# vsois/hanabi-agents

Hardware: AMD Instinct MI355X
Metric: env_steps_per_sec (higher is better)
Workload: dtype u8 env/encoder + bfloat16 Q-net GEMM (fp32 accumulate, fp32 master weights)

## Files before the change

hanabi-agents_amd/csrc/actor_fused.hip:

```cpp
#include <hip/hip_runtime.h>
#include <hip/hip_bf16.h>
#include <hip/hip_fp16.h>

#include <cstdint>
#include <type_traits>

#include "../../include/hanabi_hip.h"
#include "common.hpp"
#include "env_kernel.hpp"

using hb::fail;

namespace {

typedef __bf16 bf16x8 __attribute__((ext_vector_type(8)));
typedef _Float16 f16x8 __attribute__((ext_vector_type(8)));
typedef float f32x4 __attribute__((ext_vector_type(4)));

constexpr int FM = 128;
constexpr int FH = 512;
constexpr int FNT = 512;
constexpr int FK = 51;
constexpr int S2 = FH / 32;
constexpr int LUT_BYTES = 65536;
constexpr int H_BYTES = FM * FH * 2;
constexpr int FRAG_FLOATS = 3 * 8 * FM;
constexpr int LDS_TOTAL = H_BYTES + FRAG_FLOATS * 4;
constexpr float NEG_BIG = -1e30f;

struct FusedArgs {
  const uint32_t* obs;
  long long m;
  int words;
  int s1;
  const uint4* w1f;
  const float* b1;
  const uint4* w2f;
  const float* b2;
  const float* support;
  float* q;
  int n_actions, n_pass;
  const int8_t* legal;
  int32_t* actions;
  float epsilon;
  unsigned long long seed, draw;
  long long first_gid;
  unsigned long long* stamps;
};

#ifdef HB_STAMPS
#define HB_FSTAMP(slot)                                                                              \
  do {                                                                                               \
    __builtin_amdgcn_sched_barrier(0);                                                               \
    unsigned long long hb_t_;                                                                        \
    asm volatile("s_memtime %0\n\ts_waitcnt lgkmcnt(0)" : "=s"(hb_t_)::"memory");                    \
    if (a.stamps && lane == 0) a.stamps[(static_cast<long long>(blockIdx.x) * 8 + wave) * 16 + (slot)] = hb_t_; \
    __builtin_amdgcn_sched_barrier(0);                                                               \
  } while (0)
#define HB_FSTAMP_REAL(slot)                                                                         \
  do {                                                                                               \
    unsigned long long hb_t_;                                                                        \
    asm volatile("s_memrealtime %0\n\ts_waitcnt lgkmcnt(0)" : "=s"(hb_t_)::"memory");                \
    if (a.stamps && lane == 0) a.stamps[(static_cast<long long>(blockIdx.x) * 8 + wave) * 16 + (slot)] = hb_t_; \
  } while (0)
#else
#define HB_FSTAMP(slot) do {} while (0)
#define HB_FSTAMP_REAL(slot) do {} while (0)
#endif

template <bool F16>
__device__ __forceinline__ uint32_t pack16(float lo, float hi) {
  if constexpr (F16) {
    const _Float16 a = static_cast<_Float16>(lo), b = static_cast<_Float16>(hi);
    uint16_t ua, ub;
    __builtin_memcpy(&ua, &a, 2);
    __builtin_memcpy(&ub, &b, 2);
    return static_cast<uint32_t>(ua) | (static_cast<uint32_t>(ub) << 16);
  } else {
    const __hip_bfloat16 a = __float2bfloat16(lo), b = __float2bfloat16(hi);
    return static_cast<uint32_t>(*reinterpret_cast<const uint16_t*>(&a)) |
           (static_cast<uint32_t>(*reinterpret_cast<const uint16_t*>(&b)) << 16);
  }
}
template <bool F16>
__device__ __forceinline__ uint32_t bits2_one(uint32_t b, int p) {
  const uint32_t t = (b >> (2 * p)) & 3u;
  return __umul24((t | (t << 15)) & 0x00010001u, F16 ? 0x3C00u : 0x3F80u);
}
template <bool F16>
__device__ __forceinline__ f32x4 mfma16(const uint4& wv, const uint4& xv, const f32x4& c) {
  if constexpr (F16) {
    union { uint4 u; f16x8 f; } w, x;
    w.u = wv; x.u = xv;
    return __builtin_amdgcn_mfma_f32_16x16x32_f16(w.f, x.f, c, 0, 0, 0);
  } else {
    union { uint4 u; bf16x8 f; } w, x;
    w.u = wv; x.u = xv;
    return __builtin_amdgcn_mfma_f32_16x16x32_bf16(w.f, x.f, c, 0, 0, 0);
  }
}
typedef float f32x2 __attribute__((ext_vector_type(2)));
typedef unsigned int u32x2 __attribute__((ext_vector_type(2)));
__device__ __forceinline__ float vmax(float a, float b) {
  float r;
  asm("v_max_f32 %0, %1, %2" : "=v"(r) : "v"(a), "v"(b));
  return r;
}
__device__ __forceinline__ float vmax3(float a, float b, float c) {
  float r;
  asm("v_max3_f32 %0, %1, %2, %3" : "=v"(r) : "v"(a), "v"(b), "v"(c));
  return r;
}
__device__ __forceinline__ float exp2_fast(float x) { return __builtin_amdgcn_exp2f(x); }

template <bool F16, class K, int EG>
__device__ __forceinline__ void actor_fused_body(const FusedArgs& a) {
  __shared__ __attribute__((aligned(16))) unsigned char lds[LDS_TOTAL];
  const int tid = threadIdx.x, lane = tid & 63;
  const int wave = __builtin_amdgcn_readfirstlane(tid >> 6);
  const int r = lane & 15, qd = lane >> 4;
  const long long row0 = static_cast<long long>(blockIdx.x) * FM;
  const int s1 = a.s1, G = (s1 + 3) >> 2;
  unsigned char* lutb = lds + (LDS_TOTAL - LUT_BYTES);
  const int bits_off = LDS_TOTAL - LUT_BYTES - 2048 * G;
  unsigned char* bits = lds + bits_off;
  const int m_early = bits_off >> 14;

  HB_FSTAMP_REAL(14);
  HB_FSTAMP(0);
  const uint4* w1p = a.w1f + (4 * wave) * 64 + lane;
  uint4 wa[4], wb[4];
#pragma unroll
  for (int n = 0; n < 4; ++n) wa[n] = w1p[n * 64];

  uint32_t w[4] = {0u, 0u, 0u, 0u};
  auto load_item = [&](int it) {
    const int rr = it & (FM - 1), g = it >> 7;
    long long row = row0 + rr;
    if (row >= a.m) row = a.m - 1;
    const uint32_t* src = a.obs + row * a.words + 4 * g;
#pragma unroll
    for (int i = 0; i < 4; ++i) w[i] = (4 * g + i < a.words) ? src[i] : 0u;
  };
  if (tid < FM * G) load_item(tid);
  for (int e = tid; e < 4096; e += FNT) {
    const uint32_t v = static_cast<uint32_t>(e) >> 4;
    *reinterpret_cast<uint4*>(lutb + e * 16) = make_uint4(bits2_one<F16>(v, 0), bits2_one<F16>(v, 1), bits2_one<F16>(v, 2), bits2_one<F16>(v, 3));
  }
  for (int it = tid; it < FM * G; it += FNT) {
    const int rr = it & (FM - 1), g = it >> 7;
    if (it != tid) load_item(it);
    uint32_t* dst = reinterpret_cast<uint32_t*>(bits) + (static_cast<size_t>((rr >> 4) * G + g) * 64 + (rr & 15));
#pragma unroll
    for (int qq = 0; qq < 4; ++qq) {
      const uint32_t o = ((w[0] >> (8 * qq)) & 0xFFu) | (((w[1] >> (8 * qq)) & 0xFFu) << 8) | (((w[2] >> (8 * qq)) & 0xFFu) << 16) |
                         (((w[3] >> (8 * qq)) & 0xFFu) << 24);
      dst[qq * 16] = o;
    }
  }
  HB_FSTAMP(1);
  __syncthreads();
  HB_FSTAMP(2);

  f32x4 acc[4][8];
#pragma unroll
  for (int n = 0; n < 4; ++n) {
    const float4 b = *reinterpret_cast<const float4*>(a.b1 + 64 * wave + 16 * n + 4 * qd);
#pragma unroll
    for (int m = 0; m < 8; ++m) acc[n][m] = f32x4{b.x, b.y, b.z, b.w};
  }

  {
    const unsigned char* lut = lutb + r * 16;
    const uint32_t* bw = reinterpret_cast<const uint32_t*>(bits) + lane;
#define HB_L1_STEP(I, WCUR, WNXT, HAVE_NEXT)                                                                   \
  {                                                                                                            \
    const int s_ = 4 * g + (I);                                                                                \
    if (HAVE_NEXT) {                                                                                           \
      _Pragma("unroll") for (int n = 0; n < 4; ++n) WNXT[n] = w1p[(s_ + 1) * 2048 + n * 64];                    \
    }                                                                                                          \
    asm volatile("" ::: "memory");                \
    uint4 xf[8];                                                                                               \
    _Pragma("unroll") for (int m = 0; m < 8; ++m) {                                                            \
      const uint32_t v = (xw[m] >> (8 * (I))) & 0xFFu;                                                         \
      xf[m] = *reinterpret_cast<const uint4*>(lut + v * 256u);                                                 \
    }                                                                                                          \
    _Pragma("unroll") for (int n = 0; n < 4; ++n) {                                                            \
      _Pragma("unroll") for (int m = 0; m < 8; ++m)                                                            \
        acc[n][m] = mfma16<F16>(WCUR[n], xf[m], acc[n][m]);                                                    \
    }                                                                                                          \
  }
    for (int g = 0; g < G; ++g) {
      uint32_t xw[8];
#pragma unroll
      for (int m = 0; m < 8; ++m) xw[m] = bw[(m * G + g) * 64];
      HB_L1_STEP(0, wa, wb, true)
      const bool more = 4 * g + 2 < s1;
      HB_L1_STEP(1, wb, wa, more)
      if (more) {
        HB_L1_STEP(2, wa, wb, true)
        HB_L1_STEP(3, wb, wa, (4 * g + 4 < s1))
      }
// ... 74 lines not shown
#undef HB_L2_HALF
    if (p < 2) HB_FSTAMP(7 + 3 * p);
    if (p + 1 < n_pass) {
#pragma unroll
      for (int n = 0; n < 4; ++n) wa[n] = wp[S2 * 2048 + n * 64];
    }

    auto sup_at = [&](int k) { return a.support[k < FK ? k : FK - 1]; };
    f32x2 supF[6];
#pragma unroll
    for (int i = 0; i < 6; ++i) supF[i] = f32x2{sup_at(4 * (2 * i) + qd), sup_at(4 * (2 * i + 1) + qd)};
    const float supF12 = sup_at(48 + qd);
    const int fq = wave & 3;
    const f32x2 supZa = f32x2{sup_at(13 * fq + qd), sup_at(13 * fq + 4 + qd)};
    const f32x2 supZb = f32x2{sup_at(13 * fq + 8 + qd), sup_at(13 * fq + 12)};
    const bool full_ok = slot < A && slot < full_cap;
    float* fb = reinterpret_cast<float*>(lds + H_BYTES) + wave * FM;
    const f32x2 L2 = f32x2{LOG2E, LOG2E};
    hb::static_for<2>([&](auto MH) {
    constexpr int M0 = 4 * decltype(MH)::value;
    float qF[4], zm[4], zs[4], zt[4], vf12[4], vz3[4], nmx[4], nmz[4];
#define HB_M for (int m = 0; m < 4; ++m)
#define HB_SWAP16(X, OP) { const u32x2 t_ = __builtin_amdgcn_permlane16_swap(__float_as_uint(X), __float_as_uint(X), false, false); \
                           X = OP(__uint_as_float(t_.x), __uint_as_float(t_.y)); }
#define HB_SWAP32(X, OP) { const u32x2 t_ = __builtin_amdgcn_permlane32_swap(__float_as_uint(X), __float_as_uint(X), false, false); \
                           X = OP(__uint_as_float(t_.x), __uint_as_float(t_.y)); }
#define HB_ADD(A_, B_) ((A_) + (B_))
#pragma unroll
    HB_M { vf12[m] = qd < 3 ? acc[3][M0 + m][0] : NEG_BIG; vz3[m] = qd == 3 ? acc[3][M0 + m][0] : NEG_BIG; }
#pragma unroll
    HB_M nmx[m] = vmax3(acc[0][M0 + m][0], acc[0][M0 + m][1], acc[0][M0 + m][2]);
#pragma unroll
    HB_M nmx[m] = vmax3(nmx[m], acc[0][M0 + m][3], acc[1][M0 + m][0]);
#pragma unroll
    HB_M nmx[m] = vmax3(nmx[m], acc[1][M0 + m][1], acc[1][M0 + m][2]);
#pragma unroll
    HB_M nmx[m] = vmax3(nmx[m], acc[1][M0 + m][3], acc[2][M0 + m][0]);
#pragma unroll
    HB_M nmx[m] = vmax3(nmx[m], acc[2][M0 + m][1], acc[2][M0 + m][2]);
#pragma unroll
    HB_M nmx[m] = vmax3(nmx[m], acc[2][M0 + m][3], vf12[m]);
#pragma unroll
    HB_M nmz[m] = vmax(vmax3(acc[3][M0 + m][1], acc[3][M0 + m][2], acc[3][M0 + m][3]), vz3[m]);
#pragma unroll
    HB_M HB_SWAP16(nmx[m], vmax)
#pragma unroll
    HB_M HB_SWAP16(nmz[m], vmax)
#pragma unroll
    HB_M HB_SWAP32(nmx[m], vmax)
#pragma unroll
    HB_M HB_SWAP32(nmz[m], vmax)
#pragma unroll
    HB_M { nmx[m] *= -LOG2E; nmz[m] *= -LOG2E; }
    f32x2 s2[4], t2[4];
#define HB_PAIR_FIRST(N, LO, SUP)                                                                   \
  _Pragma("unroll") HB_M {                                                                          \
    const f32x2 arg = f32x2{acc[N][M0 + m][LO], acc[N][M0 + m][LO + 1]} * L2 + f32x2{nmx[m], nmx[m]};         \
    const f32x2 e = f32x2{exp2_fast(arg.x), exp2_fast(arg.y)};                                      \
    s2[m] = e;                                                                                      \
    t2[m] = e * SUP;                                                                                \
  }
#define HB_PAIR(N, LO, SUP)                                                                         \
  _Pragma("unroll") HB_M {                                                                          \
    const f32x2 arg = f32x2{acc[N][M0 + m][LO], acc[N][M0 + m][LO + 1]} * L2 + f32x2{nmx[m], nmx[m]};         \
    const f32x2 e = f32x2{exp2_fast(arg.x), exp2_fast(arg.y)};                                      \
    s2[m] += e;                                                                                     \
    t2[m] += e * SUP;                                                                               \
  }
    HB_PAIR_FIRST(0, 0, supF[0])
    HB_PAIR(0, 2, supF[1])
    HB_PAIR(1, 0, supF[2])
    HB_PAIR(1, 2, supF[3])
    HB_PAIR(2, 0, supF[4])
    HB_PAIR(2, 2, supF[5])
#undef HB_PAIR
#undef HB_PAIR_FIRST
    float sF[4], tF[4];
#pragma unroll
    HB_M {
      const float e12 = exp2_fast(vf12[m] * LOG2E + nmx[m]);
      sF[m] = s2[m].x + s2[m].y + e12;
      tF[m] = t2[m].x + t2[m].y + e12 * supF12;
    }
#pragma unroll
    HB_M {
      const f32x2 arg = f32x2{acc[3][M0 + m][1], acc[3][M0 + m][2]} * L2 + f32x2{nmz[m], nmz[m]};
      const f32x2 e = f32x2{exp2_fast(arg.x), exp2_fast(arg.y)};
      s2[m] = e;
      t2[m] = e * supZa;
    }
#pragma unroll
    HB_M {
      const f32x2 arg = f32x2{acc[3][M0 + m][3], vz3[m]} * L2 + f32x2{nmz[m], nmz[m]};
      const f32x2 e = f32x2{exp2_fast(arg.x), exp2_fast(arg.y)};
      s2[m] += e;
      t2[m] += e * supZb;
    }
#pragma unroll
    HB_M { zs[m] = s2[m].x + s2[m].y; zt[m] = t2[m].x + t2[m].y; }
#pragma unroll
    HB_M HB_SWAP16(sF[m], HB_ADD)
#pragma unroll
    HB_M HB_SWAP16(tF[m], HB_ADD)
#pragma unroll
    HB_M HB_SWAP16(zs[m], HB_ADD)
#pragma unroll
    HB_M HB_SWAP16(zt[m], HB_ADD)
#pragma unroll
    HB_M HB_SWAP32(sF[m], HB_ADD)
#pragma unroll
    HB_M HB_SWAP32(tF[m], HB_ADD)
#pragma unroll
    HB_M HB_SWAP32(zs[m], HB_ADD)
#pragma unroll
    HB_M HB_SWAP32(zt[m], HB_ADD)
#pragma unroll
    HB_M { zm[m] = -nmz[m]; qF[m] = tF[m] * __builtin_amdgcn_rcpf(sF[m]) * (1.0f / FK); }
#undef HB_M
#undef HB_SWAP16
#undef HB_SWAP32
#undef HB_ADD
    if (qd == 0) {
#pragma unroll
      for (int m = 0; m < 4; ++m) {
        const long long row = row0 + 16 * (M0 + m) + r;
        if (full_ok && row < a.m) a.q[row * A + slot] = qF[m];
        fb[16 * (M0 + m) + r] = zm[m];
        fb[8 * FM + 16 * (M0 + m) + r] = zs[m];
        fb[16 * FM + 16 * (M0 + m) + r] = zt[m];
      }
    }
    __builtin_amdgcn_sched_barrier(0);
    });
    if (p < 2) HB_FSTAMP(8 + 3 * p);
    __syncthreads();
    if (tid < 2 * FM) {
      const int rr = tid & (FM - 1), g = tid >> 7;
      const int ea = full_cap + 2 * p + g;
      const long long row = row0 + rr;
      if (ea < A && row < a.m) {
        const float* f = reinterpret_cast<const float*>(lds + H_BYTES) + (4 * g) * FM + rr;
        const float m0 = f[0], m1 = f[FM], m2 = f[2 * FM], m3 = f[3 * FM];
        const float M = fmaxf(fmaxf(m0, m1), fmaxf(m2, m3));
        const float e0 = exp2_fast(m0 - M), e1 = exp2_fast(m1 - M), e2 = exp2_fast(m2 - M), e3 = exp2_fast(m3 - M);
        const float* fs = f + 8 * FM;
        const float* ft = f + 16 * FM;
        const float S = fs[0] * e0 + fs[FM] * e1 + fs[2 * FM] * e2 + fs[3 * FM] * e3;
        const float T = ft[0] * e0 + ft[FM] * e1 + ft[2 * FM] * e2 + ft[3 * FM] * e3;
        a.q[row * A + ea] = T * __builtin_amdgcn_rcpf(S) * (1.0f / FK);
      }
    }
    if (p + 1 < n_pass) __syncthreads();
    if (p < 2) HB_FSTAMP(9 + 3 * p);
  }
  if (a.legal) {
    asm volatile("s_waitcnt vmcnt(0)" ::: "memory");
    __syncthreads();
    if (tid < FM && row0 + tid < a.m) {
      const long long g = row0 + tid;
      const unsigned long long gid = static_cast<unsigned long long>(a.first_gid + g);
      uint32_t rnd[4];
      hb::philox4x32_10(static_cast<uint32_t>(a.draw), static_cast<uint32_t>(a.draw >> 32), static_cast<uint32_t>(gid),
                        static_cast<uint32_t>(gid >> 32), static_cast<uint32_t>(a.seed), static_cast<uint32_t>(a.seed >> 32), rnd);
      const float* qr = a.q + g * A;
      const int8_t* lr = a.legal + g * A;
      float best = -INFINITY;
      unsigned long long legal_mask = 0, ties = 0;
      for (int i = 0; i < A; ++i) {
        const float v = __hip_atomic_load(qr + i, __ATOMIC_RELAXED, __HIP_MEMORY_SCOPE_AGENT);
        if (lr[i] != 0) {
          legal_mask |= 1ull << i;
          if (v > best) { best = v; ties = 1ull << i; }
          else if (v == best) ties |= 1ull << i;
        }
      }
      const float u = static_cast<float>(rnd[0] >> 8) * (1.0f / 16777216.0f);
      unsigned long long pool = (u < a.epsilon) ? legal_mask : ties;
      if (pool == 0) pool = legal_mask;
      int pick = 0;
      const int c = __popcll(pool);
      if (c > 0) {
        int k = static_cast<int>(__umulhi(rnd[1], static_cast<uint32_t>(c)));
        while (k-- > 0) pool &= pool - 1;
        pick = __ffsll(static_cast<long long>(pool)) - 1;
      }
      a.actions[g] = pick;
      if constexpr (!std::is_void_v<K>) reinterpret_cast<int*>(lds + H_BYTES)[tid] = pick;
    }
  }
  if constexpr (!std::is_void_v<K>) {
    constexpr int ENV_WORDS = hb::env_lds_words<K, EG>();
    static_assert((FM / EG) * ENV_WORDS * 4 <= H_BYTES && FM / EG <= FNT / 64, "env tail: the LDS slices must fit in H");
    __syncthreads();
    if (wave < FM / EG) {
#if defined(__HIP_DEVICE_COMPILE__)
      typedef const __attribute__((address_space(4))) unsigned char KargByte;
      typedef const __attribute__((address_space(4))) hb::EnvArgs KargEnv;
      auto kargs = __builtin_amdgcn_kernarg_segment_ptr();
      asm volatile("" : "+s"(kargs));
      constexpr size_t ENV_OFF = (sizeof(FusedArgs) + alignof(hb::EnvArgs) - 1) / alignof(hb::EnvArgs) * alignof(hb::EnvArgs);
      KargEnv& env = *(KargEnv*)((KargByte*)kargs + ENV_OFF);
#else
      const hb::EnvArgs env{};
#endif
      const long long g0 = row0 + EG * wave;
      const int uid = lane < EG ? reinterpret_cast<const int*>(lds + H_BYTES)[EG * wave + lane] : 0;
      hb::env_wave_step<K, EG>(env, g0, lane, reinterpret_cast<uint32_t*>(lds) + wave * ENV_WORDS, uid, g0 / EG);
    }
  }
  HB_FSTAMP_REAL(15);
}

template <bool F16>
__global__ __launch_bounds__(FNT) void actor_fused_kernel(const FusedArgs a) {
  actor_fused_body<F16, void, 16>(a);
}

template <bool F16, class K, int EG>
__global__ __launch_bounds__(FNT) void actor_env_fused_kernel(const FusedArgs a, const hb::EnvArgs env) {
  (void)env;
  actor_fused_body<F16, K, EG>(a);
}

template <bool F16>
__global__ __launch_bounds__(FNT) void actor_fused_grouped_kernel(const FusedArgs a, const hb_fused_tile* __restrict__ tiles) {
  const hb_fused_tile& t = tiles[blockIdx.x];
  if (!t.active) return;
  FusedArgs b = a;
  b.w1f = static_cast<const uint4*>(t.w1f); b.b1 = t.b1f; b.w2f = static_cast<const uint4*>(t.w2f); b.b2 = t.b2f;
  b.support = t.support;
  b.first_gid = t.first_game_id - static_cast<long long>(blockIdx.x) * FM;
  actor_fused_body<F16, void, 16>(b);
}

struct PackArgs {
  const __hip_bfloat16* w1; int w1_ld;
  const __hip_bfloat16* b1;
  const __hip_bfloat16* w2; int w2_ld;
  const __hip_bfloat16* b2;
  int obs_len, s1, n_actions, n_pass;
  uint4* w1f; float* b1f; uint4* w2f; float* b2f;
  int chunks1, chunks2;
  int f16;
  uint16_t* w1t; int w1t_ld;
  uint16_t* w2t; int w2t_ld;
};
__device__ __forceinline__ float bias_to_float(const __hip_bfloat16* b, int i, int f16) {
  return f16 ? __half2float(reinterpret_cast<const __half*>(b)[i]) : __bfloat162float(b[i]);
}
__host__ __device__ __forceinline__ int fused_logit(int col, int n_actions, int n_pass) {
  const int slot = col >> 6, c = col & 63, n = c >> 4, q = (c >> 2) & 3, j = c & 3;
  const int r16 = 4 * n + j;
  const int full_cap = 8 * n_pass;
  int action, atom;
  if (r16 < 12 || (r16 == 12 && q < 3)) {
    action = slot < full_cap ? slot : n_actions;
    if (action >= n_actions) return -1;
    atom = r16 < 12 ? 4 * r16 + q : 48 + q;
  } else {
    const int p = slot >> 3, w = slot & 7, f = w & 3;
    action = full_cap + 2 * p + (w >> 2);
    atom = r16 == 12 ? 13 * f + 12 : 13 * f + 4 * (r16 - 13) + q;
  }
  if (action >= n_actions || atom >= FK) return -1;
  return action * FK + atom;
}
__global__ __launch_bounds__(256) void actor_fused_pack_kernel(const PackArgs a) {
  const int id = static_cast<int>(blockIdx.x) * 256 + static_cast<int>(threadIdx.x);
  const __hip_bfloat16 zero = __float2bfloat16(0.f);
  if (id < a.chunks1) {
    const int lane = id & 63, nt = (id >> 6) & 31, s = id >> 11;
    const int unit = 16 * nt + (lane & 15), k0 = 32 * s + 8 * (lane >> 4);
    __hip_bfloat16 v[8];
#pragma unroll
    for (int i = 0; i < 8; ++i) v[i] = (k0 + i < a.obs_len) ? a.w1[static_cast<long long>(k0 + i) * a.w1_ld + unit] : zero;
    a.w1f[id] = *reinterpret_cast<const uint4*>(v);
    if (a.w1t) *reinterpret_cast<uint4*>(a.w1t + static_cast<size_t>(unit) * a.w1t_ld + k0) = *reinterpret_cast<const uint4*>(v);
    if (id < FH) a.b1f[id] = bias_to_float(a.b1, id, a.f16);
  } else if (id < a.chunks1 + a.chunks2) {
    const int id2 = id - a.chunks1;
    const int lane = id2 & 63, ntp = (id2 >> 6) & 31, s = (id2 >> 11) % S2, pass = (id2 >> 11) / S2;
    const int col = 16 * (32 * pass + ntp) + (lane & 15), k0 = 32 * s + 8 * (lane >> 4);
    const int lg = fused_logit(col, a.n_actions, a.n_pass);
    __hip_bfloat16 v[8];
#pragma unroll
    for (int i = 0; i < 8; ++i) v[i] = lg >= 0 ? a.w2[static_cast<long long>(k0 + i) * a.w2_ld + lg] : zero;
    a.w2f[id2] = *reinterpret_cast<const uint4*>(v);
    if (a.w2t && lg >= 0) *reinterpret_cast<uint4*>(a.w2t + static_cast<size_t>(lg) * a.w2t_ld + k0) = *reinterpret_cast<const uint4*>(v);
    if (s == 0 && (lane >> 4) == 0) a.b2f[col] = lg >= 0 ? bias_to_float(a.b2, lg, a.f16) : NEG_BIG;
  }
}

bool aligned16(const void* p) { return (reinterpret_cast<uintptr_t>(p) & 15u) == 0; }
int passes_for(int n_actions) { return (n_actions + 9) / 10; }

}

extern "C" {

int hb_actor_fused_supported(int32_t obs_len, int32_t hidden, int32_t n_actions, int32_t n_atoms) {
  return obs_len >= 1 && obs_len <= 4096 && hidden == FH && n_atoms == FK && n_actions >= 1 && n_actions <= 80 ? 1 : 0;
}

int hb_actor_fused_columns(int32_t n_actions, int32_t* phys_of_logit_host) {
  if (!phys_of_logit_host) return fail(HB_ERR_INVALID, "null argument");
  if (n_actions < 1 || n_actions > 80) return fail(HB_ERR_INVALID, "n_actions must be 1..80");
  const int np = passes_for(n_actions);
  for (int j = 0; j < n_actions * FK; ++j) phys_of_logit_host[j] = -1;
  for (int col = 0; col < 512 * np; ++col) {
    const int lg = fused_logit(col, n_actions, np);
    if (lg >= 0) phys_of_logit_host[lg] = col;
  }
  for (int j = 0; j < n_actions * FK; ++j)
    if (phys_of_logit_host[j] < 0) return fail(HB_ERR_INVALID, "internal: logit column %d has no physical column", j);
  return HB_OK;
}

int hb_actor_fused_sizes(int32_t obs_len, int32_t hidden, int32_t n_actions, int32_t n_atoms, int64_t* w1f_bytes, int64_t* w2f_bytes,
                         int32_t* b2f_floats) {
  if (!hb_actor_fused_supported(obs_len, hidden, n_actions, n_atoms)) return fail(HB_ERR_INVALID, "shape not covered by the fused actor kernel");
  const int s1 = 2 * ((obs_len + 63) / 64), np = passes_for(n_actions);
  if (w1f_bytes) *w1f_bytes = static_cast<int64_t>(32) * s1 * 64 * 16;
  if (w2f_bytes) *w2f_bytes = static_cast<int64_t>(32) * np * S2 * 64 * 16;
  if (b2f_floats) *b2f_floats = 512 * np;
  return HB_OK;
}

int hb_actor_fused_pack_dt(const void* w1_dev, int32_t w1_ld, const void* b1_dev, const void* w2_dev, int32_t w2_ld, const void* b2_dev,
                           int32_t obs_len, int32_t hidden, int32_t n_actions, int32_t n_atoms, void* w1f_dev, float* b1f_dev,
                           void* w2f_dev, float* b2f_dev, int32_t dtype, void* stream) {
  return hb_actor_fused_pack_thin(w1_dev, w1_ld, b1_dev, w2_dev, w2_ld, b2_dev, obs_len, hidden, n_actions, n_atoms, w1f_dev, b1f_dev,
                                  w2f_dev, b2f_dev, nullptr, 0, nullptr, 0, dtype, stream);
}

int hb_actor_fused_pack_thin(const void* w1_dev, int32_t w1_ld, const void* b1_dev, const void* w2_dev, int32_t w2_ld, const void* b2_dev,
                             int32_t obs_len, int32_t hidden, int32_t n_actions, int32_t n_atoms, void* w1f_dev, float* b1f_dev,
                             void* w2f_dev, float* b2f_dev, void* w1t_dev, int32_t w1t_ld, void* w2t_dev, int32_t w2t_ld,
                             int32_t dtype, void* stream) {
  if (dtype != 1 && dtype != 2) return fail(HB_ERR_INVALID, "dtype must be 1 (bf16) or 2 (f16)");
  if (!w1_dev || !b1_dev || !w2_dev || !b2_dev || !w1f_dev || !b1f_dev || !w2f_dev || !b2f_dev) return fail(HB_ERR_INVALID, "null argument");
  if (!hb_actor_fused_supported(obs_len, hidden, n_actions, n_atoms)) return fail(HB_ERR_INVALID, "shape not covered by the fused actor kernel");
  if (w1_ld < hidden || w2_ld < n_actions * n_atoms) return fail(HB_ERR_INVALID, "row strides shorter than the rows");
  if (!aligned16(w1f_dev) || !aligned16(w2f_dev)) return fail(HB_ERR_ALIGN, "w1f / w2f must be 16-byte aligned");
  PackArgs p{};
  p.w1 = static_cast<const __hip_bfloat16*>(w1_dev); p.w1_ld = w1_ld; p.b1 = static_cast<const __hip_bfloat16*>(b1_dev);
  p.w2 = static_cast<const __hip_bfloat16*>(w2_dev); p.w2_ld = w2_ld; p.b2 = static_cast<const __hip_bfloat16*>(b2_dev);
  p.obs_len = obs_len; p.s1 = 2 * ((obs_len + 63) / 64); p.n_actions = n_actions; p.n_pass = passes_for(n_actions);
  p.w1f = static_cast<uint4*>(w1f_dev); p.b1f = b1f_dev; p.w2f = static_cast<uint4*>(w2f_dev); p.b2f = b2f_dev;
  p.chunks1 = 32 * p.s1 * 64; p.chunks2 = 32 * p.n_pass * S2 * 64;
  p.f16 = dtype == 2 ? 1 : 0;
  if (w1t_dev && (w1t_ld < 32 * p.s1 || w1t_ld % 8 || !aligned16(w1t_dev))) return fail(HB_ERR_INVALID, "w1t: row stride must cover the padded K (a multiple of 8), 16-byte aligned");
  if (w2t_dev && (w2t_ld < hidden || w2t_ld % 8 || !aligned16(w2t_dev))) return fail(HB_ERR_INVALID, "w2t: row stride must cover the hidden units (a multiple of 8), 16-byte aligned");
  p.w1t = static_cast<uint16_t*>(w1t_dev); p.w1t_ld = w1t_ld; p.w2t = static_cast<uint16_t*>(w2t_dev); p.w2t_ld = w2t_ld;
  const int blocks = (p.chunks1 + p.chunks2 + 255) / 256;
  hipLaunchKernelGGL(actor_fused_pack_kernel, dim3(blocks), dim3(256), 0, static_cast<hipStream_t>(stream), p);
  HB_HIP(hipGetLastError());
  return HB_OK;
// ... 183 lines not shown
```

hanabi-agents_amd/csrc/env_api.hip:

```cpp
#include <hip/hip_runtime.h>

#include <cstdarg>
#include <cstdio>
#include <cstdlib>
#include <cstring>
#include <new>
#include <string>
#include <vector>

#include "../../include/hanabi_hip.h"
#include "common.hpp"
#include "env_kernel.hpp"

namespace hb {
const EnvVariant* variants_full(int* n);
const EnvVariant* variants_small(int* n);
const EnvVariant* variants_vsmall(int* n);

thread_local std::string g_error;
int fail(int code, const char* fmt, ...) {
  char buf[512];
  va_list ap;
  va_start(ap, fmt);
  vsnprintf(buf, sizeof buf, fmt, ap);
// ... 360 lines not shown
      unsigned seen = 0;
      for (int c = 0; c < C; ++c) seen |= m[r + c] < C ? 1u << m[r + c] : 0u;
      if (seen != (1u << C) - 1u) return fail(HB_ERR_INVALID, "row %zu of perms_dev (game %zu, seat %zu) is not a permutation of 0..%d", r / C,
                                               r / C / P, r / C % P, C - 1);
    }
  }
  hipLaunchKernelGGL(color_perms_import_kernel, dim3(static_cast<unsigned>((e->n + 255) / 256)), dim3(256), 0, st, perms_dev, e->n, P, C,
                     e->perms);
  HB_HIP(hipGetLastError());
  return HB_OK;
}

int hb_env_reset(hb_env* e, const uint8_t* mask_dev, int32_t start_player, void* stream) {
  if (!e) return fail(HB_ERR_INVALID, "null env");
  if (start_player < 0 || start_player >= e->cfg.players) return fail(HB_ERR_INVALID, "start_player out of range");
  hb::EnvArgs a{};
  a.mode = hb::MODE_RESET;
  a.mask = mask_dev;
  a.start_player = start_player;
  if (int rc = join_refill(e, stream)) return rc;
  if (int rc = refill(e, stream)) return rc;
  if (int rc = launch(e, a, stream)) return rc;
  if (int rc = draw_color_perms(e, stream)) return rc;
  return refill(e, stream);
}

int hb_env_observe(hb_env* e, int8_t* obs_dev, int8_t* legal_dev, float* agent_reward_dev, int8_t* agent_step_type_dev,
                   void* stream) {
  if (!e) return fail(HB_ERR_INVALID, "null env");
  if (int rc = check_out(obs_dev, legal_dev)) return rc;
  hb::EnvArgs a{};
  a.mode = hb::MODE_OBSERVE;
  a.obs = obs_dev;
  a.legal = legal_dev;
  a.agent_reward = agent_reward_dev;
  a.agent_step_type = agent_step_type_dev;
  return launch(e, a, stream);
}

int hb_env_step(hb_env* e, const int32_t* actions_dev, int8_t* obs_dev, int8_t* legal_dev, float* reward_dev,
                int8_t* terminal_dev, float* agent_reward_dev, int8_t* agent_step_type_dev, int8_t* score_dev,
                void* stream) {
  if (!e) return fail(HB_ERR_INVALID, "null env");
  if (!actions_dev) return fail(HB_ERR_INVALID, "actions_dev is required");
  if (int rc = check_out(obs_dev, legal_dev)) return rc;
  hb::EnvArgs a{};
  a.mode = hb::MODE_STEP;
  a.actions = actions_dev;
  a.obs = obs_dev;
  a.legal = legal_dev;
  a.reward = reward_dev;
  a.terminal = terminal_dev;
  a.agent_reward = agent_reward_dev;
  a.agent_step_type = agent_step_type_dev;
  a.score = score_dev;
  if (int rc = join_refill(e, stream)) return rc;
  if (int rc = launch(e, a, stream)) return rc;
  return refill_async(e, stream);
}

int hb_env_observe_packed(hb_env* e, uint32_t* obs_bits_dev, int8_t* obs_dev, int8_t* legal_dev, float* agent_reward_dev,
                          int8_t* agent_step_type_dev, void* stream) {
  if (!e) return fail(HB_ERR_INVALID, "null env");
  if (int rc = check_out_packed(obs_bits_dev, obs_dev, legal_dev)) return rc;
  hb::EnvArgs a{};
  a.mode = hb::MODE_OBSERVE;
  a.obs = obs_dev;
  a.obs_bits = obs_bits_dev;
  a.legal = legal_dev;
  a.agent_reward = agent_reward_dev;
  a.agent_step_type = agent_step_type_dev;
  return launch(e, a, stream);
}

int hb_env_step_packed(hb_env* e, const int32_t* actions_dev, uint32_t* obs_bits_dev, int8_t* obs_dev, int8_t* legal_dev,
                       float* reward_dev, int8_t* terminal_dev, float* agent_reward_dev, int8_t* agent_step_type_dev,
                       int8_t* score_dev, void* stream) {
  if (!e) return fail(HB_ERR_INVALID, "null env");
  if (!actions_dev) return fail(HB_ERR_INVALID, "actions_dev is required");
  if (int rc = check_out_packed(obs_bits_dev, obs_dev, legal_dev)) return rc;
  hb::EnvArgs a{};
  a.mode = hb::MODE_STEP;
  a.actions = actions_dev;
  a.obs = obs_dev;
  a.obs_bits = obs_bits_dev;
  a.legal = legal_dev;
  a.reward = reward_dev;
  a.terminal = terminal_dev;
  a.agent_reward = agent_reward_dev;
  a.agent_step_type = agent_step_type_dev;
  a.score = score_dev;
  if (int rc = join_refill(e, stream)) return rc;
  if (int rc = launch(e, a, stream)) return rc;
  return refill_async(e, stream);
}

int hb_env_step_select_packed(hb_env* e, const float* q_dev, const int8_t* sel_legal_dev, float epsilon, uint64_t seed, uint64_t draw,
                              int64_t first_game_id, int32_t* actions_out_dev, uint32_t* obs_bits_dev, int8_t* obs_dev,
                              int8_t* legal_dev, float* reward_dev, int8_t* terminal_dev, float* agent_reward_dev,
                              int8_t* agent_step_type_dev, int8_t* score_dev, void* stream) {
  if (!e) return fail(HB_ERR_INVALID, "null env");
  if (!q_dev || !sel_legal_dev || !actions_out_dev) return fail(HB_ERR_INVALID, "q_dev, sel_legal_dev and actions_out_dev are required");
  if ((reinterpret_cast<uintptr_t>(q_dev) & 15) || (reinterpret_cast<uintptr_t>(sel_legal_dev) & 3))
    return fail(HB_ERR_ALIGN, "q_dev must be 16-byte and sel_legal_dev 4-byte aligned");
  if (e->var->n_actions > 64) return fail(HB_ERR_INVALID, "the fused selection handles at most 64 actions");
  if (int rc = check_out_packed(obs_bits_dev, obs_dev, legal_dev)) return rc;
  hb::EnvArgs a{};
  a.mode = hb::MODE_STEP;
  a.sel_q = q_dev;
  a.sel_legal = sel_legal_dev;
  a.sel_actions = actions_out_dev;
  a.sel_eps = epsilon;
  a.sel_seed = seed;
  a.sel_draw = draw;
  a.sel_first_gid = first_game_id;
  a.obs = obs_dev;
  a.obs_bits = obs_bits_dev;
  a.legal = legal_dev;
  a.reward = reward_dev;
  a.terminal = terminal_dev;
  a.agent_reward = agent_reward_dev;
  a.agent_step_type = agent_step_type_dev;
  a.score = score_dev;
  if (int rc = join_refill(e, stream)) return rc;
  if (int rc = launch(e, a, stream)) return rc;
  return refill_async(e, stream);
}

int hb_actor_fused_act_step(hb_env* e, const uint32_t* obs_bits_dev, const int8_t* legal_dev, int64_t n_rows, int32_t obs_len,
                            const void* w1f_dev, const float* b1f_dev, const void* w2f_dev, const float* b2f_dev, const float* support_dev,
                            int32_t hidden, int32_t n_actions, int32_t n_atoms, float* q_dev, float epsilon, uint64_t seed, uint64_t draw,
                            int64_t first_game_id, int32_t* actions_dev, int32_t dtype, uint32_t* obs_bits_out_dev, int8_t* legal_out_dev,
                            float* reward_dev, int8_t* terminal_dev, float* agent_reward_dev, int8_t* agent_step_type_dev,
                            int8_t* score_dev, void* stream) {
  if (!e) return fail(HB_ERR_INVALID, "null env");
  if (e->shuffled) return fail(HB_ERR_INVALID, "the fused policy + env kernel has no colour-permuted form: step a shuffled env with "
                                               "hb_env_step_packed or hb_env_step_select_packed");
  if (int rc = check_out_packed(obs_bits_out_dev, nullptr, legal_out_dev)) return rc;
  hb::EnvArgs a{};
  a.mode = hb::MODE_STEP;
  a.obs_bits = obs_bits_out_dev;
  a.legal = legal_out_dev;
  a.reward = reward_dev;
  a.terminal = terminal_dev;
  a.agent_reward = agent_reward_dev;
  a.agent_step_type = agent_step_type_dev;
  a.score = score_dev;
  prepare(e, a);
  if (int rc = join_refill(e, stream)) return rc;
  if (int rc = hb::actor_env_fused_launch(obs_bits_dev, legal_dev, n_rows, obs_len, w1f_dev, b1f_dev, w2f_dev, b2f_dev, support_dev, hidden,
                                          n_actions, n_atoms, q_dev, epsilon, seed, draw, first_game_id, actions_dev, dtype, a, *e->var,
                                          stream))
    return rc;
  return refill_async(e, stream);
}

int hb_actor_fused_step_supported(const hb_env* e) { return e && !e->shuffled && hb::actor_env_fused_supported(*e->var) ? 1 : 0; }

#ifdef HB_STAMPS
int hb_env_step_stamped(hb_env* e, const int32_t* actions_dev, int8_t* obs_dev, int8_t* legal_dev,
                        unsigned long long* stamps_dev, void* stream) {
  hb::EnvArgs a{};
  a.mode = hb::MODE_STEP;
  a.actions = actions_dev;
  a.obs = obs_dev;
  a.legal = legal_dev;
  a.stamps = stamps_dev;
  if (int rc = join_refill(e, stream)) return rc;
  if (int rc = launch(e, a, stream)) return rc;
  return refill_async(e, stream);
}
#endif

int hb_env_illegal_count(hb_env* e, int64_t* out) {
  if (!e || !out) return fail(HB_ERR_INVALID, "null argument");
  unsigned long long v = 0;
  HB_HIP(hipMemcpy(&v, e->illegal, 8, hipMemcpyDeviceToHost));
  *out = static_cast<int64_t>(v);
  return HB_OK;
}

int hb_env_stats(hb_env* e, int64_t* episodes, int64_t* score_sum) {
  if (!e || !episodes || !score_sum) return fail(HB_ERR_INVALID, "null argument");
  std::vector<unsigned long long> v(static_cast<size_t>(2 * e->stat_slots));
  HB_HIP(hipMemcpy(v.data(), e->illegal + 1, 16 * e->stat_slots, hipMemcpyDeviceToHost));
  unsigned long long ep = 0, sc = 0;
  for (long long i = 0; i < e->stat_slots; ++i) { ep += v[2 * i]; sc += v[2 * i + 1]; }
  *episodes = static_cast<int64_t>(ep);
  *score_sum = static_cast<int64_t>(sc);
  return HB_OK;
}

int hb_env_set_refill_period(hb_env* e, int32_t steps) {
  if (!e) return fail(HB_ERR_INVALID, "null env");
  if (steps < 1 || steps > e->cfg.max_life) return fail(HB_ERR_INVALID, "refill period must be 1..max_life (%d)", e->cfg.max_life);
  e->refill_period = steps;
  return HB_OK;
}

int hb_env_set_async_refill(hb_env* e, int32_t on) {
  if (!e) return fail(HB_ERR_INVALID, "null env");
  HB_HIP(hipDeviceSynchronize());
  e->refill_in_flight = false;
  e->async_refill = on != 0;
  return HB_OK;
}

int hb_env_export_state(hb_env* e, uint32_t* rows_dev, void* stream) {
  if (!e || !rows_dev) return fail(HB_ERR_INVALID, "null argument");
  HB_HIP(hipMemcpyAsync(rows_dev, e->state, static_cast<size_t>(e->n) * e->var->state_words * 4, hipMemcpyDeviceToDevice,
                        static_cast<hipStream_t>(stream)));
  return HB_OK;
}
const uint32_t* hb_env_state(hb_env* e) { return e ? e->state : nullptr; }

int hb_env_import_state(hb_env* e, const uint32_t* rows_dev, void* stream) {
  if (!e || !rows_dev) return fail(HB_ERR_INVALID, "null argument");
  HB_HIP(hipMemcpyAsync(e->state, rows_dev, static_cast<size_t>(e->n) * e->var->state_words * 4, hipMemcpyDeviceToDevice,
                        static_cast<hipStream_t>(stream)));
  if (int rc = join_refill(e, stream)) return rc;
  HB_HIP(hipMemsetAsync(e->refill, 1, static_cast<size_t>(e->n), static_cast<hipStream_t>(stream)));
  if (int rc = draw_color_perms(e, stream)) return rc;
  return refill(e, stream);
}

__global__ void random_legal_kernel(const int8_t* __restrict__ legal, long long n, int n_actions, unsigned long long seed,
                                    unsigned long long draw, long long first_gid, int32_t* __restrict__ actions) {
  const long long g = static_cast<long long>(blockIdx.x) * blockDim.x + threadIdx.x;
  if (g >= n) return;
  const unsigned long long gid = static_cast<unsigned long long>(first_gid + g);
  uint32_t out[4];
  hb::philox4x32_10(static_cast<uint32_t>(draw), static_cast<uint32_t>(draw >> 32), static_cast<uint32_t>(gid),
                    static_cast<uint32_t>(gid >> 32), static_cast<uint32_t>(seed), static_cast<uint32_t>(seed >> 32), out);
  const int8_t* row = legal + g * n_actions;
  unsigned long long m = 0;
  for (int i = 0; i < n_actions; ++i) m |= static_cast<unsigned long long>(row[i] != 0) << i;
  const int n_legal = __popcll(m);
  int pick = 0;
  if (n_legal > 0) {
    int k = static_cast<int>(__umulhi(out[0], static_cast<uint32_t>(n_legal)));
    while (k-- > 0) m &= m - 1;
    pick = __ffsll(static_cast<long long>(m)) - 1;
  }
  actions[g] = pick;
}

int hb_random_legal_actions(const int8_t* legal_dev, int64_t n_games, int32_t n_actions, uint64_t seed, uint64_t draw,
                            int64_t first_game_id, int32_t* actions_dev, void* stream) {
  if (!legal_dev || !actions_dev) return fail(HB_ERR_INVALID, "null argument");
  if (n_actions < 1 || n_actions > 64) return fail(HB_ERR_INVALID, "n_actions must be 1..64");
  if (n_games <= 0) return HB_OK;
  const unsigned blocks = static_cast<unsigned>((n_games + 255) / 256);
  hipLaunchKernelGGL(random_legal_kernel, dim3(blocks), dim3(256), 0, static_cast<hipStream_t>(stream), legal_dev,
                     static_cast<long long>(n_games), n_actions, static_cast<unsigned long long>(seed),
                     static_cast<unsigned long long>(draw), static_cast<long long>(first_game_id), actions_dev);
  HB_HIP(hipGetLastError());
  return HB_OK;
}


int hb_event_create(void** event_out) {
  if (!event_out) return fail(HB_ERR_INVALID, "null event_out");
  hipEvent_t ev = nullptr;
  HB_HIP(hipEventCreateWithFlags(&ev, hipEventDisableTiming));
  *event_out = ev;
  return HB_OK;
}
int hb_event_destroy(void* event) {
  if (event) HB_HIP(hipEventDestroy(static_cast<hipEvent_t>(event)));
  return HB_OK;
}
int hb_event_record(void* event, void* stream) {
  if (!event) return fail(HB_ERR_INVALID, "null event");
  HB_HIP(hipEventRecord(static_cast<hipEvent_t>(event), static_cast<hipStream_t>(stream)));
  return HB_OK;
}
int hb_stream_wait_event(void* stream, void* event) {
  if (!event) return fail(HB_ERR_INVALID, "null event");
  HB_HIP(hipStreamWaitEvent(static_cast<hipStream_t>(stream), static_cast<hipEvent_t>(event), 0));
  return HB_OK;
}

}
```

hanabi-agents_amd/csrc/env_kernel.hpp:

```cpp
#pragma once
#include <hip/hip_runtime.h>
#include <hip/hip_ext.h>
#include <stdint.h>
#include <utility>

struct hb_config;

namespace hb {

enum { MODE_STEP = 0, MODE_OBSERVE = 1, MODE_RESET = 2 };
constexpr int NEXT_DECK_BYTES = 64;
enum { MV_PLAY = 0, MV_DISCARD = 1, MV_RCOLOR = 2, MV_RRANK = 3 };

struct EnvArgs {
  uint32_t* state;
  const int32_t* actions;
  const uint8_t* mask;
  const uint8_t* decks;
  uint8_t* next_deck;
  uint8_t* refill;
  int8_t* obs;
  uint32_t* obs_bits;
  int8_t* legal;
  float* reward;
// ... 628 lines not shown
    for (int i = 0; i < 13; ++i) row[K::W_DECK + i] = ndw[i];
    a.refill[gi] = 1;
  }
  HB_STAMP(4);
  wave_sync();
  HB_STAMP(5);

  if (active) {
    if (need_reset) {
      const uint8_t* deckb = reinterpret_cast<const uint8_t*>(row + K::W_DECK);
      w0 = static_cast<uint32_t>(K::D - P * H) | (static_cast<uint32_t>(K::INFO) << 6) | (static_cast<uint32_t>(K::LIFE) << 10) |
           (static_cast<uint32_t>(reset_start) << 13) | (static_cast<uint32_t>(P) << 16);
      w1 = 0;
      w2 = 0;
      if (!keep_seats) { w3 = 0; accw = 0; }
      w6 += 1;
      disc = 0;
#pragma unroll
      for (int p = 0; p < P; ++p) {
        uint32_t hc = 0;
        uint64_t kn = 0;
#pragma unroll
        for (int i = 0; i < 5; ++i) {
          if (i < H) {
            hc |= static_cast<uint32_t>(deckb[p * H + i]) << (5 * i);
            kn |= static_cast<uint64_t>(K::ALL_PLAUSIBLE) << (12 * i);
          } else {
            hc |= 31u << (5 * i);
          }
        }
        row[K::W_HANDS + p] = hc;
        row[K::W_KNOW + 2 * p] = static_cast<uint32_t>(kn);
        row[K::W_KNOW + 2 * p + 1] = static_cast<uint32_t>(kn >> 32);
        w1 |= static_cast<uint32_t>(H) << (15 + 3 * p);
      }
      if constexpr (SHUF) {
        const uint32_t sm = a.shuf_mask[gi];
        uint32_t e[PERM_SLOTS / 2] = {0u, 0u, 0u, 0u};
#pragma unroll
        for (int p = 0; p < P; ++p) {
          const uint32_t sg = ((sm >> p) & 1u) ? draw_perm<C>(a.seed, static_cast<unsigned long long>(a.first_gid + gi), w6, p)
                                               : identity_perm(C);
          e[p >> 1] |= sg << (16 * (p & 1));
        }
        pm = make_uint4(e[0], e[1], e[2], e[3]);
        reinterpret_cast<uint4*>(a.perms)[gi] = pm;
      }
    }
    if (mode != MODE_OBSERVE) {
      row[0] = w0; row[1] = w1; row[2] = w2; row[3] = w3;
      row[4] = static_cast<uint32_t>(accw); row[5] = static_cast<uint32_t>(accw >> 32);
      row[6] = w6; row[7] = 0;
      row[8] = static_cast<uint32_t>(disc); row[9] = static_cast<uint32_t>(disc >> 32);
    }

    if (mode != MODE_RESET) {
      const int o = (w0 >> 13) & 7;
      uint32_t sg = 0;
      if constexpr (SHUF) sg = perm_of(pm, o);
      if constexpr (LPG == 1) {
        BitAcc<K::NW> acc;
        acc.clear();
        uint64_t legal = 0;
        encode_seat<K, SHUF>(row, w0, w1, w2, disc, o, sg, acc, legal);
        uint32_t* ob = obits + lane * K::NWP;
  #pragma unroll
        for (int i = 0; i < K::NW; ++i) ob[i] = acc.w[i];
  #pragma unroll
        for (int i = K::NW; i < K::NWP; ++i) ob[i] = 0;
        uint32_t* lb = lbits + lane * K::LW;
        lb[0] = static_cast<uint32_t>(legal);
        lb[1] = static_cast<uint32_t>(legal >> 32);
        lb[2] = 0;
      }
      const uint32_t pend = (w3 >> o) & 1u, tsin = (w3 >> (5 + o)) & 1u;
      if (a.agent_reward) a.agent_reward[gi] = pend ? static_cast<float>(static_cast<int8_t>(accw >> (8 * o))) : 0.f;
      if (a.agent_step_type) a.agent_step_type[gi] = static_cast<int8_t>(!pend ? 0 : (tsin ? 2 : 1));
      if (mode == MODE_STEP) {
        if (a.reward) a.reward[gi] = out_reward;
        if (a.terminal) a.terminal[gi] = static_cast<int8_t>(out_term);
        if (a.score) a.score[gi] = static_cast<int8_t>(out_score);
      }
    }
  }
  if (mode == MODE_STEP) {
    const unsigned long long bad = __ballot(illegal);
    if (bad && lane == 0) atomicAdd(a.illegal, static_cast<unsigned long long>(__popcll(bad)));
    const unsigned long long ended = __ballot(out_term != 0);
    if (ended) {
      int sc = out_term ? out_score : 0;
      for (int o = 32; o > 0; o >>= 1) sc += __shfl_xor(sc, o);
      if (lane == 0) {
        unsigned long long* slot = a.stats + 2 * wslot;
        atomicAdd(slot, static_cast<unsigned long long>(__popcll(ended)));
        atomicAdd(slot + 1, static_cast<unsigned long long>(sc));
      }
    }
  }
  HB_STAMP(6);
  wave_sync();
  HB_STAMP(7);

  if (mode != MODE_OBSERVE) {
    constexpr int Q = K::SW / 4;
    uint4* dst = reinterpret_cast<uint4*>(a.state + g0 * K::SW);
    for (int e = lane; e < nvalid * Q; e += 64) {
      const int g = e / Q, q = e - g * Q;
      const uint32_t* s = srow + g * K::SWP + 4 * q;
      uint4 v;
      v.x = s[0]; v.y = s[1]; v.z = s[2]; v.w = s[3];
      dst[e] = v;
    }
  }
  HB_STAMP(8);
  if (mode != MODE_RESET) {
    if (a.obs_bits) {
      uint32_t* dst = a.obs_bits + g0 * K::NW;
      for (int e = lane; e < nvalid * K::NW; e += 64) {
        const int g = e / K::NW, i = e - g * K::NW;
        dst[e] = obits[g * K::NWP + i];
      }
    }
    if (a.obs) expand_rows<K::OBS_LEN>(obits, K::NWP, nvalid, a.obs + g0 * K::OBS_LEN, lane);
    expand_rows<K::A>(lbits, K::LW, nvalid, a.legal + g0 * K::A, lane);
  }
  HB_STAMP(9);
  HB_STAMP_REAL(11);
}

template <class K, int G>
__global__ __launch_bounds__(256) void env_kernel(const EnvArgs a) {
  __shared__ uint32_t lds[4 * env_lds_words<K, G>()];
  const int lane = threadIdx.x & 63;
  const int wave = threadIdx.x >> 6;
  const long long wslot = static_cast<long long>(blockIdx.x) * 4 + wave;
  const long long g0 = wslot * G;
  int uid_in = 0;
  if (a.mode == MODE_STEP && lane < G && g0 + lane < a.n) uid_in = a.sel_q ? select_action<K::A>(a, g0 + lane) : a.actions[g0 + lane];
  env_wave_step<K, G>(a, g0, lane, lds + wave * env_lds_words<K, G>(), uid_in, wslot);
}

template <class K, int G>
__global__ __launch_bounds__(256) void env_kernel_shuf(const EnvArgs a) {
  __shared__ uint32_t lds[4 * env_lds_words<K, G>()];
  const int lane = threadIdx.x & 63;
  const int wave = threadIdx.x >> 6;
  const long long wslot = static_cast<long long>(blockIdx.x) * 4 + wave;
  const long long g0 = wslot * G;
  int uid_in = 0;
  if (a.mode == MODE_STEP && lane < G && g0 + lane < a.n) uid_in = a.sel_q ? select_action<K::A>(a, g0 + lane) : a.actions[g0 + lane];
  env_wave_step<K, G, true>(a, g0, lane, lds + wave * env_lds_words<K, G>(), uid_in, wslot);
}

template <class K>
__global__ __launch_bounds__(256) void refill_kernel(const EnvArgs a) {
  constexpr int GR = 16;
  const int lane = threadIdx.x & 63;
  const long long g0 = (static_cast<long long>(blockIdx.x) * 4 + (threadIdx.x >> 6)) * GR;
  if (g0 >= a.n) return;
  const long long gi = g0 + lane;
  const bool mine = lane < GR && gi < a.n && a.refill[gi] != 0;
  unsigned long long todo = __ballot(mine);
  while (todo) {
    const int src = __ffsll(static_cast<long long>(todo)) - 1;
    todo &= todo - 1;
    const long long g = g0 + src;
    uint8_t* dst = a.next_deck + g * NEXT_DECK_BYTES;
    if (a.decks) {
      if (lane < K::D) dst[lane] = a.decks[g * K::D + lane];
    } else {
      const uint32_t episode = a.state[g * K::SW + 6];
      const unsigned long long gid = static_cast<unsigned long long>(a.first_gid + g);
      uint32_t out[4];
      philox4x32_10(static_cast<uint32_t>(lane), episode, static_cast<uint32_t>(gid), static_cast<uint32_t>(gid >> 32),
                    static_cast<uint32_t>(a.seed), static_cast<uint32_t>(a.seed >> 32), out);
      const uint32_t key = (out[0] & ~63u) | static_cast<uint32_t>(lane);
      int rank = 0;
      static_for<K::D>([&](auto I) {
        constexpr int i = decltype(I)::value;
        const uint32_t ki = static_cast<uint32_t>(__builtin_amdgcn_readlane(static_cast<int>(key), i));
        rank += ki < key ? 1 : 0;
      });
      if (lane < K::D) {
        const int col = lane / K::CPC, k = lane - col * K::CPC;
        const int rk = k < 3 ? 0 : 1 + (k - 3) / 2;
        dst[rank] = static_cast<uint8_t>(col * K::R + rk);
      }
    }
  }
  if (mine) a.refill[gi] = 0;
}

template <class K>
void launch_refill(const EnvArgs& a, hipStream_t stream) {
  const unsigned blocks = static_cast<unsigned>((a.n + 63) / 64);
  if (blocks == 0) return;
  hipLaunchKernelGGL((refill_kernel<K>), dim3(blocks), dim3(256), 0, stream, a);
}

template <class K, int G>
void launch_env(const EnvArgs& a, hipStream_t stream) {
  const long long per_block = 4LL * G;
  const unsigned blocks = static_cast<unsigned>((a.n + per_block - 1) / per_block);
  if (blocks == 0) return;
  if (a.ev_start && a.ev_stop)
    hipExtLaunchKernelGGL((env_kernel<K, G>), dim3(blocks), dim3(256), 0, stream, a.ev_start, a.ev_stop, 0, a);
  else
    hipLaunchKernelGGL((env_kernel<K, G>), dim3(blocks), dim3(256), 0, stream, a);
}

template <class K, int G>
void launch_env_shuf(const EnvArgs& a, hipStream_t stream) {
  const long long per_block = 4LL * G;
  const unsigned blocks = static_cast<unsigned>((a.n + per_block - 1) / per_block);
  if (blocks == 0) return;
  if (a.ev_start && a.ev_stop)
    hipExtLaunchKernelGGL((env_kernel_shuf<K, G>), dim3(blocks), dim3(256), 0, stream, a.ev_start, a.ev_stop, 0, a);
  else
    hipLaunchKernelGGL((env_kernel_shuf<K, G>), dim3(blocks), dim3(256), 0, stream, a);
}

struct EncodeArgs {
  const uint32_t* rows;
  uint32_t* obs_bits;
  int8_t* obs;
  int8_t* legal;
  long long n;
  int seat;
};

template <class K, int G>
__global__ __launch_bounds__(256) void encode_rows_kernel(const EncodeArgs a) {
  __shared__ uint32_t lds[4 * env_lds_words<K, G>()];
  const int lane = threadIdx.x & 63;
  const int wave = threadIdx.x >> 6;
  const long long g0 = (static_cast<long long>(blockIdx.x) * 4 + wave) * G;
  uint32_t* const srow = lds + wave * env_lds_words<K, G>();
  uint32_t* const obits = srow + G * K::SWP;
  uint32_t* const lbits = obits + G * K::NWP;
  const long long left = a.n - g0;
  if (left <= 0) return;
  const int nvalid = left < G ? static_cast<int>(left) : G;
  {
    constexpr int Q = K::SW / 4;
    constexpr int ROUNDS = (G * Q + 63) / 64;
    const uint4* src = reinterpret_cast<const uint4*>(a.rows + g0 * K::SW);
    uint4 v[ROUNDS];
#pragma unroll
    for (int r = 0; r < ROUNDS; ++r) {
      const int e = lane + 64 * r;
      v[r] = e < nvalid * Q ? src[e] : make_uint4(0u, 0u, 0u, 0u);
    }
#pragma unroll
    for (int r = 0; r < ROUNDS; ++r) {
      const int e = lane + 64 * r;
      if (e < nvalid * Q) {
        const int g = e / Q, q = e - g * Q;
        uint32_t* d = srow + g * K::SWP + 4 * q;
        d[0] = v[r].x; d[1] = v[r].y; d[2] = v[r].z; d[3] = v[r].w;
      }
    }
  }
  wave_sync();
  if (lane < nvalid) {
    const uint32_t* row = srow + lane * K::SWP;
    const uint32_t w0 = row[0], w1 = row[1], w2 = row[2];
    const uint64_t disc = (static_cast<uint64_t>(row[9]) << 32) | row[8];
    const int cur = (w0 >> 13) & 7;
    const int o = a.seat < 0 ? cur : a.seat;
    BitAcc<K::NW> acc;
    acc.clear();
    uint64_t legal = 0;
    encode_seat<K, false>(row, w0, w1, w2, disc, o, 0u, acc, legal);
    if (o != cur) legal = 0;
    uint32_t* ob = obits + lane * K::NWP;
#pragma unroll
    for (int i = 0; i < K::NW; ++i) ob[i] = acc.w[i];
#pragma unroll
    for (int i = K::NW; i < K::NWP; ++i) ob[i] = 0;
    uint32_t* lb = lbits + lane * K::LW;
    lb[0] = static_cast<uint32_t>(legal);
    lb[1] = static_cast<uint32_t>(legal >> 32);
    lb[2] = 0;
  }
  wave_sync();
  if (a.obs_bits) {
    uint32_t* dst = a.obs_bits + g0 * K::NW;
    for (int e = lane; e < nvalid * K::NW; e += 64) {
      const int g = e / K::NW, i = e - g * K::NW;
      dst[e] = obits[g * K::NWP + i];
    }
  }
  if (a.obs) expand_rows<K::OBS_LEN>(obits, K::NWP, nvalid, a.obs + g0 * K::OBS_LEN, lane);
  if (a.legal) expand_rows<K::A>(lbits, K::LW, nvalid, a.legal + g0 * K::A, lane);
}

template <class K, int G>
void launch_encode(const EncodeArgs& a, hipStream_t stream) {
  const long long per_block = 4LL * G;
  const unsigned blocks = static_cast<unsigned>((a.n + per_block - 1) / per_block);
  if (blocks == 0) return;
  hipLaunchKernelGGL((encode_rows_kernel<K, G>), dim3(blocks), dim3(256), 0, stream, a);
}

using LaunchFn = void (*)(const EnvArgs&, hipStream_t);
using EncodeFn = void (*)(const EncodeArgs&, hipStream_t);
struct EnvVariant {
  int P, C, R, H, INFO, LIFE;
  int obs_len, n_actions, deck, state_words;
  LaunchFn g8, g16, g32, g64, refill;
  LaunchFn s8, s16, s32, s64;
  EncodeFn e16, e32;
};

template <class K>
constexpr EnvVariant make_variant() {
  return EnvVariant{K::P, K::C, K::R, K::H, K::INFO, K::LIFE, K::OBS_LEN, K::A, K::D, K::SW,
                    &launch_env<K, 8>, &launch_env<K, 16>, &launch_env<K, 32>, &launch_env<K, 64>, &launch_refill<K>,
                    &launch_env_shuf<K, 8>, &launch_env_shuf<K, 16>, &launch_env_shuf<K, 32>, &launch_env_shuf<K, 64>,
                    &launch_encode<K, 16>, &launch_encode<K, 32>};
}

const EnvVariant* find_variant(const ::hb_config* c);

bool actor_env_fused_supported(const EnvVariant& v);
int actor_env_fused_launch(const uint32_t* obs_bits_dev, const int8_t* legal_dev, int64_t n_rows, int32_t obs_len, const void* w1f_dev,
                           const float* b1f_dev, const void* w2f_dev, const float* b2f_dev, const float* support_dev, int32_t hidden,
                           int32_t n_actions, int32_t n_atoms, float* q_dev, float epsilon, uint64_t seed, uint64_t draw,
                           int64_t first_game_id, int32_t* actions_dev, int32_t dtype, const EnvArgs& env, const EnvVariant& var,
                           void* stream);

}
```

Before: 316.7 million.

## Fuse deck refill into the actor-env fused kernel, dropping the separate refill launch

```diff
diff --git a/hanabi-agents_amd/csrc/actor_fused.hip b/hanabi-agents_amd/csrc/actor_fused.hip
--- a/hanabi-agents_amd/csrc/actor_fused.hip
+++ b/hanabi-agents_amd/csrc/actor_fused.hip
@@ -48,6 +48,18 @@
   unsigned long long* stamps;
 };
 
+#if defined(__HIP_DEVICE_COMPILE__)
+typedef const __attribute__((address_space(4))) unsigned char KargByte;
+typedef const __attribute__((address_space(4))) hb::EnvArgs KargEnv;
+constexpr size_t ENV_KARG_OFF = (sizeof(FusedArgs) + alignof(hb::EnvArgs) - 1) / alignof(hb::EnvArgs) * alignof(hb::EnvArgs);
+#define HB_ENV_KARGS(NAME)                                            \
+  auto NAME##_kargs_ = __builtin_amdgcn_kernarg_segment_ptr();        \
+  asm volatile("" : "+s"(NAME##_kargs_));                             \
+  KargEnv& NAME = *(KargEnv*)((KargByte*)NAME##_kargs_ + ENV_KARG_OFF)
+#else
+#define HB_ENV_KARGS(NAME) const hb::EnvArgs NAME{}
+#endif
+
 #ifdef HB_STAMPS
 #define HB_FSTAMP(slot)                                                                              \
   do {                                                                                               \
@@ -428,6 +440,20 @@
     }
     if (p + 1 < n_pass) __syncthreads();
     if (p < 2) HB_FSTAMP(9 + 3 * p);
+  }
+  [[maybe_unused]] uint32_t rf_flag[2] = {0u, 0u}, rf_ep[2] = {0u, 0u};
+  if constexpr (!std::is_void_v<K>) {
+    if (wave >= 2) {
+      HB_ENV_KARGS(env);
+#pragma unroll
+      for (int h = 0; h < 2; ++h) {
+        const long long g = row0 + 64 * h + lane;
+        if (g < env.n) {
+          rf_flag[h] = env.refill[g];
+          rf_ep[h] = env.state[g * K::SW + 6];
+        }
+      }
+    }
   }
   if (a.legal) {
     asm volatile("s_waitcnt vmcnt(0)" ::: "memory");
@@ -465,20 +491,34 @@
     }
   }
   if constexpr (!std::is_void_v<K>) {
+    static_assert(K::LIFE >= 2, "a deck flagged by one launch is regenerated by the next: a game must outlive the step after its deal");
+    if (wave >= 2) {
+      HB_ENV_KARGS(env);
+      int turn = wave - 2;
+#pragma unroll
+      for (int h = 0; h < 2; ++h) {
+        unsigned long long todo = __ballot(rf_flag[h] != 0u);
+        while (todo) {
+          const int src = __ffsll(static_cast<long long>(todo)) - 1;
+          todo &= todo - 1;
+          if (turn == 0) {
+            const long long g = row0 + 64 * h + src;
+            hb::refill_deck<K>(env, g, lane, [&] {
+              return static_cast<uint32_t>(__builtin_amdgcn_readlane(static_cast<int>(rf_ep[h]), src));
+            });
+            if (lane == 0) env.refill[g] = 0;
+            turn = 6;
+          }
+          --turn;
+        }
+      }
+      asm volatile("s_waitcnt vmcnt(0)" ::: "memory");
+    }
     constexpr int ENV_WORDS = hb::env_lds_words<K, EG>();
     static_assert((FM / EG) * ENV_WORDS * 4 <= H_BYTES && FM / EG <= FNT / 64, "env tail: the LDS slices must fit in H");
     __syncthreads();
     if (wave < FM / EG) {
-#if defined(__HIP_DEVICE_COMPILE__)
-      typedef const __attribute__((address_space(4))) unsigned char KargByte;
-      typedef const __attribute__((address_space(4))) hb::EnvArgs KargEnv;
-      auto kargs = __builtin_amdgcn_kernarg_segment_ptr();
-      asm volatile("" : "+s"(kargs));
-      constexpr size_t ENV_OFF = (sizeof(FusedArgs) + alignof(hb::EnvArgs) - 1) / alignof(hb::EnvArgs) * alignof(hb::EnvArgs);
-      KargEnv& env = *(KargEnv*)((KargByte*)kargs + ENV_OFF);
-#else
-      const hb::EnvArgs env{};
-#endif
+      HB_ENV_KARGS(env);
       const long long g0 = row0 + EG * wave;
       const int uid = lane < EG ? reinterpret_cast<const int*>(lds + H_BYTES)[EG * wave + lane] : 0;
       hb::env_wave_step<K, EG>(env, g0, lane, reinterpret_cast<uint32_t*>(lds) + wave * ENV_WORDS, uid, g0 / EG);
diff --git a/hanabi-agents_amd/csrc/env_api.hip b/hanabi-agents_amd/csrc/env_api.hip
--- a/hanabi-agents_amd/csrc/env_api.hip
+++ b/hanabi-agents_amd/csrc/env_api.hip
@@ -536,7 +536,8 @@
                                           n_actions, n_atoms, q_dev, epsilon, seed, draw, first_game_id, actions_dev, dtype, a, *e->var,
                                           stream))
     return rc;
-  return refill_async(e, stream);
+  e->since_refill = 1;
+  return HB_OK;
 }
 
 int hb_actor_fused_step_supported(const hb_env* e) { return e && !e->shuffled && hb::actor_env_fused_supported(*e->var) ? 1 : 0; }
diff --git a/hanabi-agents_amd/csrc/env_kernel.hpp b/hanabi-agents_amd/csrc/env_kernel.hpp
--- a/hanabi-agents_amd/csrc/env_kernel.hpp
+++ b/hanabi-agents_amd/csrc/env_kernel.hpp
@@ -804,6 +804,32 @@
   env_wave_step<K, G, true>(a, g0, lane, lds + wave * env_lds_words<K, G>(), uid_in, wslot);
 }
 
+template <class K, class EpisodeFn>
+__device__ __forceinline__ void refill_deck(const EnvArgs& a, long long g, int lane, EpisodeFn&& episode_of) {
+  uint8_t* dst = a.next_deck + g * NEXT_DECK_BYTES;
+  if (a.decks) {
+    if (lane < K::D) dst[lane] = a.decks[g * K::D + lane];
+  } else {
+    const uint32_t episode = episode_of();
+    const unsigned long long gid = static_cast<unsigned long long>(a.first_gid + g);
+    uint32_t out[4];
+    philox4x32_10(static_cast<uint32_t>(lane), episode, static_cast<uint32_t>(gid), static_cast<uint32_t>(gid >> 32),
+                  static_cast<uint32_t>(a.seed), static_cast<uint32_t>(a.seed >> 32), out);
+    const uint32_t key = (out[0] & ~63u) | static_cast<uint32_t>(lane);
+    int rank = 0;
+    static_for<K::D>([&](auto I) {
+      constexpr int i = decltype(I)::value;
+      const uint32_t ki = static_cast<uint32_t>(__builtin_amdgcn_readlane(static_cast<int>(key), i));
+      rank += ki < key ? 1 : 0;
+    });
+    if (lane < K::D) {
+      const int col = lane / K::CPC, k = lane - col * K::CPC;
+      const int rk = k < 3 ? 0 : 1 + (k - 3) / 2;
+      dst[rank] = static_cast<uint8_t>(col * K::R + rk);
+    }
+  }
+}
+
 template <class K>
 __global__ __launch_bounds__(256) void refill_kernel(const EnvArgs a) {
   constexpr int GR = 16;
@@ -817,28 +843,7 @@
     const int src = __ffsll(static_cast<long long>(todo)) - 1;
     todo &= todo - 1;
     const long long g = g0 + src;
-    uint8_t* dst = a.next_deck + g * NEXT_DECK_BYTES;
-    if (a.decks) {
-      if (lane < K::D) dst[lane] = a.decks[g * K::D + lane];
-    } else {
-      const uint32_t episode = a.state[g * K::SW + 6];
-      const unsigned long long gid = static_cast<unsigned long long>(a.first_gid + g);
-      uint32_t out[4];
-      philox4x32_10(static_cast<uint32_t>(lane), episode, static_cast<uint32_t>(gid), static_cast<uint32_t>(gid >> 32),
-                    static_cast<uint32_t>(a.seed), static_cast<uint32_t>(a.seed >> 32), out);
-      const uint32_t key = (out[0] & ~63u) | static_cast<uint32_t>(lane);
-      int rank = 0;
-      static_for<K::D>([&](auto I) {
-        constexpr int i = decltype(I)::value;
-        const uint32_t ki = static_cast<uint32_t>(__builtin_amdgcn_readlane(static_cast<int>(key), i));
-        rank += ki < key ? 1 : 0;
-      });
-      if (lane < K::D) {
-        const int col = lane / K::CPC, k = lane - col * K::CPC;
-        const int rk = k < 3 ? 0 : 1 + (k - 3) / 2;
-        dst[rank] = static_cast<uint8_t>(col * K::R + rk);
-      }
-    }
+    refill_deck<K>(a, g, lane, [&] { return a.state[g * K::SW + 6]; });
   }
   if (mine) a.refill[gi] = 0;
 }
```

Measured after the change: 321.3 million, median of 6. +1.5%, better.
